# uclasystem/dorylus

Measured on AMD Instinct MI355X. Metric: full-graph GCN epoch: aggregated edges/sec (epoch time in ms_per_step), Reddit-scale synthetic, 2-layer 602-128-41, higher is better.
Workload: dtype f32

## Files before the change

dorylus_amd/_lib.py:

```python
import ctypes as C
import os

import numpy as np

_HERE = os.path.dirname(os.path.abspath(__file__))
LIB_PATH = os.environ.get("DORY_LIB_PATH") or os.path.join(_HERE, "libdorylus_hip.so")

SYMBOLS = [
    "dory_create", "dory_destroy", "dory_last_error", "dory_set_streams", "dory_sync",
    "dory_configure", "dory_graph_upload", "dory_preallocate", "dory_tensor_info",
    "dory_tensor_upload", "dory_tensor_download", "dory_tensor_fill_uniform", "dory_labels_upload",
    "dory_weight_set", "dory_weight_get", "dory_weight_grad_get", "dory_weight_grad_set", "dory_weights_init_xavier",
    "dory_aggregate", "dory_apply_vertex", "dory_apply_edge", "dory_predict_gat", "dory_train_stat", "dory_train_stat_global",
    "dory_halo_plan", "dory_comm_unique_id", "dory_comm_init", "dory_halo_exchange", "dory_halo_pack",
    "dory_halo_unpack", "dory_halo_pack_tensor", "dory_halo_unpack_tensor", "dory_adam_config", "dory_weight_update", "dory_timing_enable",
    "dory_timing_get", "dory_timing_reset", "dory_set_option", "dory_get_option", "dory_ctx_describe",
    "dory_epoch_graph_begin", "dory_epoch_graph_end", "dory_epoch_graph_launch", "dory_epoch_graph_drop",
    "dory_gatmh_heads", "dory_transform_first_active", "dory_transform_first_layer",
    "dory_comm_set_host_transport", "dory_comm_init_local", "dory_debug_occupy_cus",
]

ALLTOALLV_FN = C.CFUNCTYPE(C.c_int, C.c_void_p, C.POINTER(C.c_float), C.POINTER(C.c_uint64), C.POINTER(C.c_uint64),
                           C.POINTER(C.c_float), C.POINTER(C.c_uint64), C.POINTER(C.c_uint64), C.c_uint32)
ALLREDUCE_FN = C.CFUNCTYPE(C.c_int, C.c_void_p, C.POINTER(C.c_float), C.c_uint64)
# ... 56 lines not shown
        "dory_get_option": [vp, cp, C.POINTER(C.c_int64)],
        "dory_transform_first_active": [vp],
        "dory_transform_first_layer": [vp, u32],
        "dory_epoch_graph_begin": [vp], "dory_epoch_graph_end": [vp], "dory_epoch_graph_launch": [vp, u32],
        "dory_epoch_graph_drop": [vp],
        "dory_ctx_describe": [vp, C.POINTER(i32), C.POINTER(u32), C.POINTER(u32), C.POINTER(u32), C.POINTER(u32)],
        "dory_gatmh_heads": [vp, vp],
        "dory_comm_set_host_transport": [vp, ALLTOALLV_FN, ALLREDUCE_FN, vp],
        "dory_comm_init_local": [vp, C.c_uint32],
        "dory_partition_build": [vp, vp, u64, vp, u32, u32, u32, i32, C.POINTER(vp)],
        "dory_partition_build_from_files": [cp, u32, u32, i32, C.POINTER(vp)],
        "dory_partition_load": [cp, C.POINTER(vp)],
        "dory_partition_save": [vp, cp],
        "dory_partition_free": [vp],
        "dory_partition_get": [vp, vp],
        "dory_partition_upload": [vp, vp, vp],
        "dory_partition_recv_plan": [vp, vp, i32, vp, vp],
        "dory_partition_wire_order": [vp, vp, i32, vp, vp],
        "dory_read_layer_config": [cp, vp, u32, C.POINTER(u32)],
        "dory_read_features": [cp, vp, u32, u32, cp, vp, vp],
        "dory_read_labels": [cp, vp, u32, vp],
        "dory_engine_create": [vp, C.POINTER(vp)],
        "dory_engine_destroy": [vp],
        "dory_engine_run": [vp, u32, vp],
        "dory_engine_nn_compute": [vp, vp],
        "dory_engine_inc_layer": [vp, vp, vp],
        "dory_chunk_inc_layer": [i32, u32, vp, vp],
        "dory_engine_trace_epoch": [i32, u32, C.c_char_p, C.c_size_t],
        "dory_engine_is_last_layer": [vp, vp],
        "dory_engine_report": [vp, cp, C.c_size_t],
        "dory_sweep_deal": [u32, u32, u32, vp, vp, vp],
        "dory_sweep_deal_weighted": [u32, vp, u32, u32, u32, vp, vp, vp],
        "dory_sweep_geometry": [u32, u32, i32, i32, i32, u32, u32, u32, i32, vp],
    }
    for name, args in sig.items():
        if name in ("dory_partition_wire_order", "dory_sweep_geometry") and not hasattr(lib, name):
            continue
        fn = getattr(lib, name)
        fn.argtypes = args
        fn.restype = i32
    lib.dory_last_error.argtypes = [vp]
    lib.dory_last_error.restype = cp
    lib.dory_host_last_error.argtypes = []
    lib.dory_host_last_error.restype = cp
    lib.dory_formats_last_error.argtypes = []
    lib.dory_formats_last_error.restype = cp
    return lib


def _ptr(a):
    return a.ctypes.data_as(C.c_void_p) if a is not None else None


class Context:

    def __init__(self, device=0, lib=None):
        self.lib = lib or load()
        h = C.c_void_p()
        rc = self.lib.dory_create(device, C.byref(h))
        if rc != 0:
            raise DoryError(f"dory_create failed ({rc}): {self.lib.dory_last_error(None).decode()}")
        self.h = h
        self._keep = []

    def _ck(self, rc):
        if rc != 0:
            raise DoryError(f"dorylus_hip error {rc}: {self.lib.dory_last_error(self.h).decode()}")

    def close(self):
# ... 247 lines not shown
```

dorylus_amd/csrc/abi_context.hip:

```cpp
#include "abi_internal.hpp"

namespace dory {

static std::string g_create_err;

int fail(dory_ctx *c, int code, const char *fmt, ...) {
    char buf[512];
    va_list ap;
    va_start(ap, fmt);
    vsnprintf(buf, sizeof(buf), fmt, ap);
    va_end(ap);
    if (c) c->err = buf; else g_create_err = buf;
    return code;
}

void drain_timing(dory_ctx *c) {
    const dory_ctx::Pending *halo = nullptr;
    for (auto &p : c->pending) {
        (void)hipEventSynchronize(p.b);
        float ms = 0.f;
        if (hipEventElapsedTime(&ms, p.a, p.b) == hipSuccess) {
            c->times[p.fam].total_ms += ms;
            c->times[p.fam].launches += 1;
        }
// ... 156 lines not shown
int dory_create(int device, dory_ctx **out) {
    if (!out) return DORY_ERR_ARG;
    int n = 0;
    if (hipGetDeviceCount(&n) != hipSuccess || n == 0)
        return fail(nullptr, DORY_ERR_NODEVICE, "no HIP device visible (this library has no CPU fallback)");
    if (device < 0 || device >= n) return fail(nullptr, DORY_ERR_ARG, "device %d out of range (%d)", device, n);
    hipDeviceProp_t prop;
    if (hipGetDeviceProperties(&prop, device) != hipSuccess)
        return fail(nullptr, DORY_ERR_HIP, "hipGetDeviceProperties failed");
    if (!strstr(prop.gcnArchName, "gfx950"))
        return fail(nullptr, DORY_ERR_NODEVICE, "device %d is %s; kernels are built for gfx950 only", device,
                    prop.gcnArchName);
    dory_ctx *c = new dory_ctx();
    c->device = device;
    if (hipSetDevice(device) != hipSuccess || hipStreamCreateWithFlags(&c->compute, hipStreamNonBlocking) != hipSuccess ||
        hipStreamCreateWithFlags(&c->comm, hipStreamNonBlocking) != hipSuccess ||
        hipEventCreateWithFlags(&c->ev_a, hipEventDisableTiming) != hipSuccess ||
        hipEventCreateWithFlags(&c->ev_b, hipEventDisableTiming) != hipSuccess ||
        hipMalloc((void **)&c->d_stat, 2 * sizeof(float)) != hipSuccess ||
        hipMalloc((void **)&c->sweep_stat, SWEEP_STAT_WORDS * sizeof(uint32_t)) != hipSuccess ||
        hipMalloc((void **)&c->d_stat3, 256) != hipSuccess) {
        delete c;
        return fail(nullptr, DORY_ERR_HIP, "stream/event creation failed");
    }
    (void)hipMemset(c->d_stat, 0, 2 * sizeof(float));
    (void)hipMemset(c->sweep_stat, 0, SWEEP_STAT_WORDS * sizeof(uint32_t));
    c->own_compute = c->own_comm = true;
    c->opt["spmm_variant"] = 2;
    c->opt["spmm_sweep_flags"] = 0;
    c->opt["spmm_sweep_rows"] = 0;
    c->opt["spmm_sweep_pair"] = -1;
    c->opt["spmm_sweep_loader"] = 1;
    c->opt["spmm_sweep_loader_relief"] = 3;
    c->opt["spmm_sweep_reserve_cus"] = 4;
    c->opt["spmm_sweep_layout"] = 3;
    c->opt["spmm_sweep_window_kb"] = 0;
    c->cus_per_xcd = (uint32_t)std::max(1, prop.multiProcessorCount / 8);
    {
        const uint32_t PG = 2048;
        uint32_t *dx = nullptr;
        std::vector<uint32_t> hx(PG, 0xFFu);
        if (hipMalloc((void **)&dx, PG * sizeof(uint32_t)) == hipSuccess) {
            bool ran = launch_xcd_probe(dx, PG, c->compute) == hipSuccess && hipStreamSynchronize(c->compute) == hipSuccess &&
                       hipMemcpy(hx.data(), dx, PG * sizeof(uint32_t), hipMemcpyDeviceToHost) == hipSuccess;
            (void)hipFree(dx);
            uint32_t seen = 0, match = 0;
            for (uint32_t i = 0; i < PG; ++i) { if (hx[i] < 16) seen |= 1u << hx[i]; match += hx[i] == hx[i & 7u]; }
            uint32_t firsts = 0;
            for (uint32_t r = 0; r < 8; ++r) if (hx[r] < 16) firsts |= 1u << hx[r];
            c->xcd_count = (uint32_t)__builtin_popcount(seen);
            c->xcd_mapping_ok = ran && match == PG && c->xcd_count == 8 && __builtin_popcount(firsts) == 8;
        } else {
            c->xcd_mapping_ok = false;
        }
    }
    c->opt["spmm_xcd_assume_mismatch"] = 0;
    c->opt["spmm_slab"] = 0;
    c->opt["spmm_order"] = 1;
    c->opt["spmm_blk_group"] = 32;
    c->opt["spmm_blk_force_split"] = 0;
    c->opt["halo_overlap"] = 1;
    c->opt["gat_lazy_edge_tensors"] = 1;
    c->opt["gat_reuse_nsum"] = 1;
    c->opt["spmm_edge_split"] = 1;
    c->opt["spmm_sweep_cus"] = 0;
    c->opt["local_timeout_ms"] = 30000;
// ... 789 lines not shown
```

dorylus_amd/csrc/abi_stages.hip:

```cpp
#include "abi_internal.hpp"

namespace dory {
static BlockedAdj &gatmh_blocked_for(Adjacency &A, uint32_t ld) { return ld < 128 && A.blk16.built ? A.blk16 : A.blk; }

int ensure_blocked(dory_ctx *c, Adjacency &A, int group, bool narrow_set) {
    DerivedAdj &B = narrow_set ? A.blk16 : A.blk;
    const uint32_t want_nb = (uint32_t)c->opt["spmm_blk_nb"];
    const bool rebuild = B.built && want_nb && B.nb != (want_nb + 7) / 8 * 8;
    if (c->capturing && (!B.built || rebuild) && !A.blk.na)
        return fail(c, DORY_ERR_ARG, "epoch graph: blocked adjacency would have to be (re)built while recording");
    if (rebuild) {
        HIPCK(c, hipStreamSynchronize(c->compute));
        free_blocked(&B);
        B.built = false;
    }
    if (!B.built) {
        const uint32_t NG = c->N + A.ghosts;
        const uint64_t window = 0;
        const uint32_t nb = plan_blocks(NG, want_nb, (uint32_t)group * 16u, window);
        const bool tiny = !want_nb && (uint64_t)NG * group * 16u <= ((uint64_t)4 << 20) &&
                          !(c->gnn == DORY_GATMH && c->numNodes > 1);
        if (tiny || nb > 256 || (uint64_t)nb * (c->N + 1) * 8ull > ((uint64_t)8 << 30)) {
            if (!narrow_set) A.blk.na = true;
            return DORY_OK;
// ... 5 lines not shown
    return DORY_OK;
}

int ensure_sweep(dory_ctx *c, Adjacency &A, int group) {
    DerivedAdj &S = A.swp;
    const uint32_t want_nb = (uint32_t)c->opt["spmm_blk_nb"];
    if (S.built && S.want_nb != want_nb && !c->capturing) {
        HIPCK(c, hipStreamSynchronize(c->compute));
        free_blocked(&S);
        S.built = false;
    }
    if (S.built || S.na) return DORY_OK;
    if (c->capturing) return fail(c, DORY_ERR_ARG, "epoch graph: the sweep layout would have to be built while recording");
    const uint32_t NG = c->N + A.ghosts;
    int R;
    if (c->gnn == DORY_GATMH) {
        const uint32_t G_ = std::min<uint32_t>(32u, c->cus_per_xcd);
        const int forced = (int)c->opt["gatmh_sweep_rows"];
        R = (!forced && c->N >= 8u * G_ * 32u * 4u) ? 4 : sweep_pick_r(c->N, 32, G_, forced, 4);
    } else {
        R = sweep_pick_r(c->N, 32, std::min<uint32_t>(32u, c->cus_per_xcd), (int)c->opt["spmm_sweep_rows"]);
    }
    const bool out_edges = &A == &c->adj[ADJ_OUT];
    const uint64_t gat_kb = (c->gnn == DORY_GATMH && out_edges && c->opt["gatmh_src_window_kb"]) ? (uint64_t)c->opt["gatmh_src_window_kb"] : 4608u;
    const uint64_t window_kb = c->opt["spmm_sweep_window_kb"] ? (uint64_t)c->opt["spmm_sweep_window_kb"]
                                                              : (c->gnn == DORY_GATMH && R >= 4 ? gat_kb : (R <= 4 ? 3584u : 2432u));
    const uint64_t window = window_kb << 10;
    const uint64_t nb_est = ((uint64_t)NG * group * 16u + window - 1) / window + 1;
    const bool tiny = !want_nb && (uint64_t)NG * group * 16u <= ((uint64_t)4 << 20);
    if (tiny || c->N < 8 || (want_nb ? want_nb : nb_est) > 512 || (want_nb ? want_nb : nb_est) * (uint64_t)(c->N + 1) * 8ull > ((uint64_t)8 << 30)) {
        S.na = true;
        return DORY_OK;
    }
    HIPCK(c, build_blocked_sweep(A.ptr, A.idx, A.val, c->N, NG, A.nnz, want_nb, (uint32_t)group * 16u, window, R, &S, c->compute,
                                 (uint32_t)c->opt["spmm_sweep_layout"], std::min<uint32_t>(32u, c->cus_per_xcd),
                                 group == 32 && c->opt["spmm_sweep_loader"] ? (uint32_t)c->opt["spmm_sweep_loader_relief"] : 0u));
    S.want_nb = want_nb;
    S.built = true;
    return DORY_OK;
}

int blk_group_for(dory_ctx *c, uint32_t ld) {
    int group = (int)c->opt["spmm_blk_group"];
    if (group != 8 && group != 16 && group != 32) group = 32;
    if (ld < 128 && group == 32) group = 16;
    return group;
}

static int bf16_reserve(dory_ctx *c, uint64_t rows, uint32_t ld, const char *option) {
    const size_t need = (size_t)rows * ld * sizeof(uint16_t);
    if (need <= c->bf16_rows_bytes) return DORY_OK;
    if (c->capturing) return fail(c, DORY_ERR_ARG, "epoch graph: the bf16 rows of %s would have to grow while recording", option);
    if (c->bf16_rows) {
        HIPCK(c, hipStreamSynchronize(c->compute));
        (void)hipFree(c->bf16_rows);
        c->bf16_rows = nullptr;
        c->bf16_rows_bytes = 0;
        epoch_graph_drop_locked(c);
    }
    HIPCK(c, hipMalloc((void **)&c->bf16_rows, need));
    c->bf16_rows_bytes = need;
    return DORY_OK;
}
static int bf16_convert(dory_ctx *c, const Tensor &t, uint64_t first_row) {
    if (!t.rows) return DORY_OK;
    Timed tc(c, "bf16_convert", c->compute);
    HIPCK(c, launch_bf16_rows(t.d, c->bf16_rows + first_row * t.ld, t.rows * t.ld, c->compute));
    return DORY_OK;
}
// ... 775 lines not shown
```

dorylus_amd/csrc/ctx.hpp:

```cpp
#pragma once
#include <hip/hip_runtime.h>

#include <atomic>
#include <cstdint>
#include <map>
#include <memory>
#include <mutex>
#include <string>
#include <vector>

#include "../../include/dorylus_hip.h"
#include "sweep_geometry.hpp"

namespace dory {

struct Tensor {
    uint64_t rows = 0;
    uint32_t cols = 0;
    uint32_t ld = 0;
    float *d = nullptr;
    bool owned = true;
    size_t bytes() const { return (size_t)rows * ld * sizeof(float); }
};

// ... 210 lines not shown
    uint32_t N;
    uint32_t F;
    uint32_t ld;
    const uint64_t *ptr;
    const uint32_t *idx;
    const float *val;
    const float *self_scale;
    int self_mode;
    const float *xl;
    const float *xg;
    float *out;
    int accumulate;
    uint32_t row_clamp;
    uint32_t rows;
    const uint32_t *order;
    const uint64_t *ptr_end;
};
hipError_t launch_spmm(const SpmmArgs &a, int slab, hipStream_t s, bool bf16 = false);

void plan_long_rows(const uint64_t *ptr, uint32_t N, LongRowsHost *out);
hipError_t launch_spmm_long_rows(const SpmmArgs &a, const LongRowsDev &L, float *partial , hipStream_t s, bool bf16 = false);

hipError_t build_blocked(const uint64_t *ptr, const uint32_t *idx, const float *val, uint32_t N, uint32_t NG,
                         uint64_t nnz, uint32_t want_nb , uint32_t row_bytes, BlockedAdj *out,
                         hipStream_t s, uint64_t window_bytes = 0 );
uint32_t plan_blocks(uint32_t NG, uint32_t want_nb, uint32_t row_bytes, uint64_t window_bytes = 0);
hipError_t launch_spmm_blocked_part(const SpmmArgs &a, const BlockedAdj &B, float *partial, int group, bool unit,
                                    uint32_t b_lo, uint32_t b_hi, hipStream_t s);
hipError_t launch_spmm_blocked_long_segments(const SpmmArgs &a, const BlockedAdj &B, float *partial, bool unit,
                                             float *chunk_partial , hipStream_t s);
hipError_t launch_spmm_blocked_reduce(const SpmmArgs &a, const BlockedAdj &B, const float *partial,
                                      const float *row_scale, hipStream_t s);
void free_blocked(BlockedAdj *B);
hipError_t build_blocked_sweep(const uint64_t *ptr, const uint32_t *idx, const float *val, uint32_t N, uint32_t NG,
                               uint64_t nnz, uint32_t want_nb, uint32_t row_bytes, uint64_t window_bytes, int R,
                               BlockedAdj *out, hipStream_t s, uint32_t layout = 3 ,
                               uint32_t sweep_tiles = 32 ,
                               uint32_t loader_relief = 0 );
bool sweep_deal_plan(uint32_t nl, uint32_t R, uint32_t sweep_tiles, std::vector<uint32_t> *cap, uint32_t *npos, uint32_t loader_relief = 0);
bool sweep_deal_positions(uint32_t nl, uint32_t R, const std::vector<uint32_t> &cap, uint32_t *pos, uint32_t loader_lo = 0);
bool sweep_deal_balanced(uint32_t nl, uint32_t R, const std::vector<uint32_t> &cap, const uint64_t *w, uint32_t *pos);
int sweep_pick_r(uint32_t N, int group, uint32_t G, int force_r = 0 , int max_r = 10);
int sweep_rows(uint32_t rows_per_group, uint32_t npos, int group, uint32_t G, int force_r );
bool sweep_wide_rows_ok(int R);
SweepGeometry sweep_geometry(uint32_t npos, uint32_t ld, int group, int R, bool wide, uint32_t G);
size_t sweep_counter_bytes(const SweepGeometry &g, uint32_t nblocks);
size_t sweep_counter_bound(uint32_t npos, uint32_t ld, int group, int R, bool wide, uint32_t G, uint32_t nblocks);
bool sweep_supported(const SpmmArgs &a, const BlockedAdj &B, int group);
struct SweepCtl {
    int pair = -1;
    bool loader = true;
    uint32_t *stat = nullptr;
};
constexpr int SWEEP_STAT_WORDS = 8;
struct SweepPart {
    uint32_t cus;
    uint32_t b_lo, b_hi;
    bool accumulate;
    uint32_t reserve;
    int R;
    uint32_t *done;
    SweepCtl ctl;
    uint32_t flags;
    hipStream_t s;
    bool bf16;
    bool wide;
};
inline bool sweep_wide_applies(uint32_t ld, int group, int R16) { return ld >= 128 && (group == 16 || group == 32) && sweep_wide_rows_ok(R16); }
hipError_t launch_spmm_sweep(SpmmArgs a, const BlockedAdj &B, int group, const float *row_scale, float *split_partial, const SweepPart &p);
hipError_t launch_spmm_sweep_combine(const SpmmArgs &a, const BlockedAdj &B, const float *row_scale, const float *split_partial,
                                     hipStream_t s, bool bf16 = false);
hipError_t launch_bf16_rows(const float *x, uint16_t *y, uint64_t n, hipStream_t s);
hipError_t launch_occupy_cus(uint32_t workgroups, uint64_t usec, hipStream_t s);
hipError_t launch_xcd_probe(uint32_t *xcc , uint32_t grid, hipStream_t s);
// ... 159 lines not shown
```

dorylus_amd/csrc/spmm.hip:

```cpp
#include <algorithm>
#include <cmath>
#include <vector>

#include "sweep_core.hpp"

namespace dory {

template <int GROUP, int CHUNKS, bool BF16>
__device__ __forceinline__ void spmm_rows_body(SpmmArgs a) {
    typedef RowChunk<BF16> RC;
    constexpr int RPW = 64 / GROUP;
    constexpr int RPB = 4 * RPW;
    const int lane = threadIdx.x & 63;
    const int wave = threadIdx.x >> 6;
    const int li = lane % GROUP;
    const int gi = lane / GROUP;
    const uint32_t rid = blockIdx.x * RPB + wave * RPW + gi;
    const bool row_ok = rid < (a.rows ? a.rows : a.N);
    uint32_t v = row_ok ? (a.order ? a.order[rid] : rid) : 0;
    if constexpr (GROUP == 64)
        v = (uint32_t)__builtin_amdgcn_readfirstlane((int)v);

    const uint32_t nchunk = a.ld >> 2;
    const uint32_t c0 = blockIdx.y * (GROUP * CHUNKS) + li;
    bool act[CHUNKS];
    uint32_t col[CHUNKS];
    float4 acc[CHUNKS];
#pragma unroll
    for (int k = 0; k < CHUNKS; ++k) {
        act[k] = row_ok && (c0 + GROUP * k) < nchunk;
        col[k] = act[k] ? c0 + GROUP * k : 0;
        acc[k] = make_float4(0.f, 0.f, 0.f, 0.f);
    }
    if (a.accumulate == 2) {
// ... 342 lines not shown
        }
        if (a.self_mode != 0) {
            const float sc = a.self_mode == 1 ? a.self_scale[v] : 1.f;
            acc = fma4(sc, row_chunk(xl4[(size_t)v * nchunk + col]), acc);
        }
        if (a.accumulate) {
            const float4 p = out4[col];
            acc.x += p.x; acc.y += p.y; acc.z += p.z; acc.w += p.w;
        }
        out4[col] = acc;
    }
}
__global__ __launch_bounds__(320) void spmm_sweep_combine_kernel(SpmmArgs a, BlockedAdj B, const float *row_scale,
                                                                 const float *split_partial, uint32_t tpr) {
    spmm_sweep_combine_body<false>(a, B, row_scale, split_partial, tpr);
}
__global__ __launch_bounds__(320) void spmm_sweep_combine_bf16_kernel(SpmmArgs a, BlockedAdj B, const float *row_scale,
                                                                      const float *split_partial, uint32_t tpr) {
    spmm_sweep_combine_body<true>(a, B, row_scale, split_partial, tpr);
}

hipError_t launch_spmm_sweep_combine(const SpmmArgs &a, const BlockedAdj &B, const float *row_scale, const float *split_partial,
                                     hipStream_t s, bool bf16) {
    if (!B.nsplit || a.ld == 0) return hipSuccess;
    const uint32_t nchunk = a.ld >> 2;
    const uint32_t tpr = std::min<uint32_t>(256u, (nchunk + 31u) & ~31u);
    const uint32_t rpb = std::max<uint32_t>(1u, 320u / tpr);
    hipLaunchKernelGGL(bf16 ? spmm_sweep_combine_bf16_kernel : spmm_sweep_combine_kernel, dim3((B.nsplit + rpb - 1) / rpb),
                       dim3(tpr * rpb), 0, s, a, B, row_scale, split_partial, tpr);
    return hipGetLastError();
}

constexpr uint32_t SWEEP_SPLIT = 2;

hipError_t build_blocked_sweep(const uint64_t *ptr, const uint32_t *idx, const float *val, uint32_t N, uint32_t NG,
                               uint64_t nnz, uint32_t want_nb, uint32_t row_bytes, uint64_t window_bytes, int R,
                               BlockedAdj *out, hipStream_t s, uint32_t layout, uint32_t sweep_tiles, uint32_t loader_relief) {
    BlockedAdj B{};
    if (N == 0 || NG == 0) { *out = B; return hipSuccess; }
    hipError_t e;
#define BCK(x) if ((e = (x)) != hipSuccess) return e
    std::vector<uint64_t> hptr((size_t)N + 1);
    BCK(hipMemcpyAsync(hptr.data(), ptr, ((size_t)N + 1) * sizeof(uint64_t), hipMemcpyDeviceToHost, s));
    BCK(hipStreamSynchronize(s));
    const uint64_t split_deg = std::max<uint64_t>(64, (uint64_t)SWEEP_SPLIT * (nnz / N + 1));
    struct Item { uint32_t row, k, K; uint64_t w; };
    std::vector<Item> items;
    items.reserve(N);
    std::vector<uint32_t> split_rows;
    uint32_t nslots = 0;
    for (uint32_t v = 0; v < N; ++v) {
        const uint64_t deg = hptr[v + 1] - hptr[v];
        if (deg > split_deg) {
            const uint64_t K64 = (deg + split_deg - 1) / split_deg;
            if (K64 > 0x7FFFFFFFull || (uint64_t)nslots + K64 > 0x7FFFFFFFull) return hipErrorInvalidValue;
            const uint32_t K = (uint32_t)K64;
            split_rows.insert(split_rows.end(), {v, nslots, K});
            for (uint32_t k = 0; k < K; ++k) items.push_back({v, k, K, (deg + K - 1) / K});
            nslots += K;
        } else {
            items.push_back({v, 0, 1, deg});
        }
    }
    if (layout & 2u) std::stable_sort(items.begin(), items.end(), [](const Item &x, const Item &y) { return x.w > y.w; });
    const uint64_t ni64 = items.size();
    if (ni64 + 16 > 0xFFFFFFF0ull) return hipErrorInvalidValue;
    const uint32_t nl = (uint32_t)ni64;
    uint32_t npos = std::max<uint32_t>((nl + R - 1) / (uint32_t)R * (uint32_t)R, 8);
    std::vector<uint32_t> ipos(nl);
    if (layout & 2u) {
// ... 53 lines not shown
    B.SB = (std::max(N, G) + std::max(nbL, std::max<uint32_t>(nbG, 1)) - 1) / std::max(nbL, std::max<uint32_t>(nbG, 1));
    B.npos = npos;
    B.nb_local = nbL;
    B.nghost = G;
    B.rows_per_group = (uint32_t)R;
    B.row_bytes = row_bytes;
    uint32_t *cnt = nullptr;
    uint16_t *d_sblk = nullptr;
    uint64_t *dtotal = nullptr;
    BCK(hipMalloc((void **)&B.perm, (size_t)npos * sizeof(uint32_t)));
    BCK(hipMemcpyAsync(B.perm, perm.data(), (size_t)npos * sizeof(uint32_t), hipMemcpyHostToDevice, s));
    BCK(hipMalloc((void **)&d_sblk, (size_t)NG * sizeof(uint16_t)));
    BCK(hipMemcpyAsync(d_sblk, sblk.data(), (size_t)NG * sizeof(uint16_t), hipMemcpyHostToDevice, s));
    uint2 *d_slice = nullptr;
    if (nslots) {
        BCK(hipMalloc((void **)&B.otgt, (size_t)npos * sizeof(uint32_t)));
        BCK(hipMemcpyAsync(B.otgt, otgt.data(), (size_t)npos * sizeof(uint32_t), hipMemcpyHostToDevice, s));
        BCK(hipMalloc((void **)&d_slice, (size_t)npos * sizeof(uint2)));
        BCK(hipMemcpyAsync(d_slice, slice.data(), (size_t)npos * sizeof(uint2), hipMemcpyHostToDevice, s));
        BCK(hipMalloc((void **)&B.split_rows, split_rows.size() * sizeof(uint32_t)));
        BCK(hipMemcpyAsync(B.split_rows, split_rows.data(), split_rows.size() * sizeof(uint32_t), hipMemcpyHostToDevice, s));
        B.nsplit = (uint32_t)(split_rows.size() / 3);
        B.nslots = nslots;
    }
    BCK(hipMalloc((void **)&cnt, (size_t)nb * npos * sizeof(uint32_t)));
    BCK(hipMemsetAsync(cnt, 0, (size_t)nb * npos * sizeof(uint32_t), s));
    BCK(hipMalloc((void **)&B.boff, (size_t)nb * (npos + 1) * sizeof(uint32_t)));
    BCK(hipMalloc((void **)&B.bbase, (size_t)(nb + 1) * sizeof(uint64_t)));
    BCK(hipMalloc((void **)&B.bent, (nnz + 130) * sizeof(uint2)));
    BCK(hipMemsetAsync(B.bent + nnz, 0, 130 * sizeof(uint2), s));
    BCK(hipMalloc((void **)&dtotal, nb * sizeof(uint64_t)));
    hipLaunchKernelGGL(blk_count_kernel, dim3((npos + 255) / 256), dim3(256), 0, s, npos, ptr, idx, B.SB, cnt, B.perm, d_sblk,
                       (const uint2 *)d_slice);
    hipLaunchKernelGGL(blk_scan_kernel, dim3(nb), dim3(1024), 0, s, npos, cnt, B.boff, dtotal);
    std::vector<uint64_t> tot(nb), base(nb + 1, 0);
    BCK(hipMemcpyAsync(tot.data(), dtotal, nb * sizeof(uint64_t), hipMemcpyDeviceToHost, s));
    BCK(hipStreamSynchronize(s));
    for (uint32_t b = 0; b < nb; ++b) base[b + 1] = base[b] + tot[b];
    if (base[nb] != nnz) return hipErrorUnknown;
    BCK(hipMemcpyAsync(B.bbase, base.data(), (nb + 1) * sizeof(uint64_t), hipMemcpyHostToDevice, s));
    hipLaunchKernelGGL(blk_fill_kernel, dim3((npos + 255) / 256), dim3(256), 0, s, npos, nb, ptr, idx, val, B.SB, B.bbase,
                       B.boff, cnt, (uint32_t *)nullptr, (float *)nullptr, B.perm, d_sblk, (const uint2 *)d_slice, B.bent);
    BCK(hipGetLastError());
    BCK(hipStreamSynchronize(s));
    (void)hipFree(cnt);
    (void)hipFree(dtotal);
    (void)hipFree(d_sblk);
    if (d_slice) (void)hipFree(d_slice);
#undef BCK
    *out = B;
    return hipSuccess;
}

bool sweep_supported(const SpmmArgs &a, const BlockedAdj &B, int group) {
    const uint64_t row_b = (uint64_t)a.ld * 4u;
    const bool addr_ok = (uint64_t)a.N * row_b < (1ull << 32) && (uint64_t)B.nghost * row_b < (1ull << 32) &&
                         (uint64_t)a.N + B.nghost < (1u << 24) && row_b < (1u << 24);
    return (group == 16 || group == 32) && !(a.ld & 3) && B.nb > 0 && B.nchunks == 0 && a.N >= 8 && B.npos >= 8 && addr_ok;
}

hipError_t sweep_plan(const SpmmArgs &a, const BlockedAdj &B, int group, const SweepPart &p, float *split_partial, SweepPlan *pl) {
    if (!sweep_supported(a, B, group) || p.b_hi > B.nb || p.cus == 0 || p.cus > 32 || !p.ctl.stat) return hipErrorInvalidValue;
    if (p.b_lo < B.nb_local && p.b_hi > B.nb_local) return hipErrorInvalidValue;
    if (p.b_lo >= B.nb_local && !a.xg) return hipErrorInvalidValue;
    const uint32_t G = p.cus > 12 ? p.cus - std::min<uint32_t>(p.reserve, 8u) : p.cus;
    const SweepGeometry g = sweep_geometry(B.npos, a.ld, group, p.R, p.wide, G);
    const uint32_t flags = p.flags | (p.accumulate ? 2u : 0u) | (p.reserve ? 32u : 0u);
    *pl = SweepPlan{SweepArgs{g.rpx, g.tiles_x, G, g.nsweeps, p.b_lo, p.b_hi, p.done, flags, split_partial, p.ctl.stat}, dim3(g.grid_x), g.slabs};
    return hipMemsetAsync(p.done, 0, sweep_counter_bytes(g, p.b_hi - p.b_lo), p.s);
}

template <class F>
static bool k1s_narrow_form(int group, int R, F f) {
    if (group == 32) return sweep_pick<2, 4, 6, 8, 10>(R, [&](auto RR) { return f(std::integral_constant<int, 32>{}, RR); });
    return group == 16 && sweep_pick<2, 3, 4, 5, 6, 8>(R, [&](auto RR) { return f(std::integral_constant<int, 16>{}, RR); });
}

hipError_t launch_spmm_sweep(SpmmArgs a, const BlockedAdj &B, int group, const float *row_scale, float *split_partial, const SweepPart &p) {
    if (a.N == 0 || a.ld == 0 || p.b_lo >= p.b_hi) return hipSuccess;
    if (p.bf16 && row_scale) return hipErrorInvalidValue;
    if (p.wide && (!p.bf16 || (a.ld & 7) || !sweep_wide_applies(a.ld, group, p.R))) return hipErrorInvalidValue;
    if (B.nslots && !split_partial) return hipErrorInvalidValue;
    if (p.accumulate) { a.self_mode = 0; a.accumulate = 1; }
    SweepPlan pl;
    const hipError_t e = sweep_plan(a, B, group, p, split_partial, &pl);
    if (e != hipSuccess) return e;
    const dim3 bl(SWEEP_NT);
    const bool unit = row_scale != nullptr;
    const bool pair = (p.R & 1) ? false : (p.ctl.pair < 0 ? pl.slabs >= 3 : p.ctl.pair != 0);
    const bool found = p.wide ? sweep_pick<2, 3, 4, 5>(p.R, [&](auto R) {
        return sweep_pick<0, 1>(p.ctl.loader, [&](auto L) {
            hipLaunchKernelGGL((spmm_sweep_bf16x8_kernel<R(), L() != 0>), pl.grid, bl, 0, p.s, a, B, pl.w);
            return true;
        });
    }) : k1s_narrow_form(group, p.R, [&](auto G, auto R) {
        return sweep_pick<0, 1>(p.ctl.loader, [&](auto L) {
            return sweep_pick<0, 1>(pair, [&](auto P) {
                hipLaunchKernelGGL((p.bf16 ? spmm_sweep_bf16_kernel<G(), R(), false, P() != 0, L() != 0>
                                    : unit ? spmm_sweep_kernel<G(), R(), true, P() != 0, L() != 0>
                                           : spmm_sweep_kernel<G(), R(), false, P() != 0, L() != 0>), pl.grid, bl, 0, p.s, a, B, row_scale, pl.w);
                return true;
            });
        });
    });
    return found ? hipGetLastError() : hipErrorInvalidValue;
}

__global__ __launch_bounds__(1024) void occupy_cus_kernel(uint64_t ticks, uint32_t *sink) {
    extern __shared__ uint32_t occupy_lds[];
    asm volatile("v_mov_b32 v127, 0" ::: "v127");
    const uint64_t t0 = wall_clock64();
    while (wall_clock64() - t0 < ticks) __builtin_amdgcn_s_sleep(64);
    if (ticks == ~0ull) { occupy_lds[threadIdx.x] = 1; sink[0] = occupy_lds[0]; }
}
hipError_t launch_occupy_cus(uint32_t workgroups, uint64_t usec, hipStream_t s) {
    if (!workgroups) return hipSuccess;
    hipError_t e = hipFuncSetAttribute(reinterpret_cast<const void *>(occupy_cus_kernel), hipFuncAttributeMaxDynamicSharedMemorySize, 96 << 10);
    if (e != hipSuccess) return e;
    hipLaunchKernelGGL(occupy_cus_kernel, dim3(workgroups), dim3(1024), 96 << 10, s, usec * 100ull, (uint32_t *)nullptr);
    return hipGetLastError();
}

// ... 11 lines not shown
```

dorylus_amd/host/sweep_deal.cpp:

```cpp
#include <algorithm>
#include <cstdint>
#include <vector>

#include "../../include/dorylus_host.h"

namespace dory {

bool sweep_deal_plan(uint32_t nl, uint32_t R, uint32_t sweep_tiles, std::vector<uint32_t> *cap, uint32_t *npos,
                     uint32_t loader_relief) {
    if (R == 0) return false;
    loader_relief = std::min(loader_relief, R / 2);
    const uint32_t tiles = std::max<uint32_t>(1, sweep_tiles);
    const uint32_t GS = tiles * 32u;
    const uint32_t n_x = (nl + 7) / 8;
    auto relief_of = [&](uint32_t rows) { return (uint32_t)(((uint64_t)loader_relief * rows + R / 2) / R); };
    auto capacity = [&](uint32_t need) -> uint64_t {
        const uint32_t S = (need + R - 1) / R, last = need - (S - 1) * R;
        const uint64_t full = (uint64_t)GS * R - (uint64_t)2 * tiles * relief_of(R);
        const uint64_t tail = (uint64_t)GS * last - (uint64_t)2 * tiles * std::min(relief_of(last), last);
        return (uint64_t)(S - 1) * full + tail;
    };
    uint32_t need = std::max<uint32_t>(1, (n_x + GS - 1) / GS);
    const uint32_t S_plain = (need + R - 1) / R;
    for (;; --loader_relief) {
        need = std::max<uint32_t>(1, (n_x + GS - 1) / GS);
        while (capacity(need) < n_x) ++need;
        if ((need + R - 1) / R == S_plain || loader_relief == 0) break;
    }
    const uint32_t S = (need + R - 1) / R;
    if ((uint64_t)8 * S * GS * R > 0xFFFFFFF0ull) return false;
    const uint32_t T = 8u * S * GS;
    const uint32_t last = need - (S - 1) * R;
    cap->assign(T, R);
    for (uint32_t x = 0; x < 8; ++x)
// ... 37 lines not shown
    }
    return i == nl;
}

bool sweep_deal_balanced(uint32_t nl, uint32_t R, const std::vector<uint32_t> &cap, const uint64_t *w, uint32_t *pos) {
    const uint32_t T = (uint32_t)cap.size();
    struct Node { uint64_t load; uint32_t cap, g; };
    auto worse = [](const Node &a, const Node &b) {
        const unsigned __int128 l = (unsigned __int128)a.load * b.cap, r = (unsigned __int128)b.load * a.cap;
        return l != r ? l > r : a.g > b.g;
    };
    std::vector<Node> heap;
    heap.reserve(T);
    for (uint32_t g = 0; g < T; ++g)
        if (cap[g]) heap.push_back({0, cap[g], g});
    std::make_heap(heap.begin(), heap.end(), worse);
    std::vector<uint32_t> used(T, 0);
    for (uint32_t i = 0; i < nl; ++i) {
        if (heap.empty()) return false;
        std::pop_heap(heap.begin(), heap.end(), worse);
        Node n = heap.back();
        heap.pop_back();
        if (used[n.g] >= R) return false;
        pos[i] = n.g * R + used[n.g]++;
        n.load += w[i];
        if (used[n.g] < cap[n.g]) {
            heap.push_back(n);
            std::push_heap(heap.begin(), heap.end(), worse);
        }
    }
    return heap.empty();
}

}

extern "C" int dory_sweep_deal(uint32_t items, uint32_t rows_per_group, uint32_t sweep_tiles, uint32_t *positions_out,
                               uint32_t *group_rows_out, uint32_t *item_position) {
    std::vector<uint32_t> cap;
    uint32_t npos = 0;
    if (!dory::sweep_deal_plan(items, rows_per_group, sweep_tiles, &cap, &npos, 0)) return 1;
    if (positions_out) *positions_out = npos;
    if (group_rows_out) std::copy(cap.begin(), cap.end(), group_rows_out);
    if (item_position && !dory::sweep_deal_positions(items, rows_per_group, cap, item_position, 0)) return 2;
    return 0;
}

extern "C" int dory_sweep_deal_weighted(uint32_t items, const uint64_t *weights, uint32_t rows_per_group, uint32_t sweep_tiles,
                                        uint32_t loader_relief, uint32_t *positions_out, uint32_t *group_rows_out,
                                        uint32_t *item_position) {
    if (!weights) return 1;
    std::vector<uint32_t> cap;
    uint32_t npos = 0;
    if (!dory::sweep_deal_plan(items, rows_per_group, sweep_tiles, &cap, &npos, loader_relief)) return 1;
    if (positions_out) *positions_out = npos;
    if (group_rows_out) std::copy(cap.begin(), cap.end(), group_rows_out);
    if (item_position && !dory::sweep_deal_balanced(items, rows_per_group, cap, weights, item_position)) return 2;
    return 0;
}
```

include/dorylus_host.h:

```cpp
#ifndef DORYLUS_HOST_H
#define DORYLUS_HOST_H

#include <stddef.h>
#include <stdint.h>

#include "dorylus_hip.h"

#ifdef __cplusplus
extern "C" {
#endif

typedef struct dory_partition dory_partition;

int dory_partition_build(const uint32_t *src, const uint32_t *dst, uint64_t num_records,
                         const int32_t *parts, uint32_t global_vtx_cnt, uint32_t node_id,
                         uint32_t num_nodes, int undirected, dory_partition **out);
int dory_partition_build_from_files(const char *dataset_dir, uint32_t node_id, uint32_t num_nodes,
                                    int undirected, dory_partition **out);
int dory_partition_load(const char *graph_bin_path, dory_partition **out);
int dory_partition_save(const dory_partition *p, const char *graph_bin_path);
int dory_partition_free(dory_partition *p);
const char *dory_host_last_error(void);

struct dory_partition_view {
// ... 21 lines not shown

int dory_partition_wire_order(const dory_partition *p, const int32_t *parts, int dir, uint32_t *order, uint32_t *idxs);

int dory_partition_upload(dory_ctx *ctx, const dory_partition *p, const int32_t *parts);

int dory_read_layer_config(const char *path, uint32_t *dims, uint32_t max_dims, uint32_t *count);
int dory_read_features(const char *path, const dory_partition *p, uint32_t expect_dim, uint32_t node_id,
                       const char *cache_dir, float *local, float *ghost);
int dory_read_labels(const char *path, const dory_partition *p, uint32_t expect_kinds, uint32_t *labels);
const char *dory_formats_last_error(void);

typedef struct dory_engine dory_engine;
int dory_engine_create(dory_ctx *ctx, dory_engine **out);
int dory_engine_destroy(dory_engine *e);
int dory_engine_run(dory_engine *e, uint32_t epochs, double *epoch_ms);
struct dory_chunk {
    uint32_t localId, globalId, lowBound, upBound, layer;
    int32_t dir;
    uint32_t epoch;
    uint8_t vertex;
};
int dory_engine_nn_compute(dory_engine *e, struct dory_chunk *chunk);
int dory_engine_inc_layer(dory_engine *e, const struct dory_chunk *in, struct dory_chunk *out);
int dory_engine_is_last_layer(dory_engine *e, const struct dory_chunk *c);
int dory_chunk_inc_layer(int gnn_type, uint32_t num_layers, const struct dory_chunk *in, struct dory_chunk *out);
int dory_engine_trace_epoch(int gnn_type, uint32_t num_layers, char *buf, size_t buflen);
int dory_engine_report(dory_engine *e, char *buf, size_t buflen);

int dory_sweep_deal(uint32_t items, uint32_t rows_per_group, uint32_t sweep_tiles, uint32_t *positions_out,
                    uint32_t *group_rows_out, uint32_t *item_position);
int dory_sweep_deal_weighted(uint32_t items, const uint64_t *weights, uint32_t rows_per_group, uint32_t sweep_tiles,
                             uint32_t loader_relief, uint32_t *positions_out, uint32_t *group_rows_out,
                             uint32_t *item_position);
int dory_sweep_geometry(uint32_t positions, uint32_t ld, int group, int rows, int wide, uint32_t cus, uint32_t nblocks,
                        uint32_t layout_rows, int rows_option, uint64_t *out);

#ifdef __cplusplus
}
#endif
#endif
```

Before: 18.91 billion.

## Rearrange sweep SpMM row positions within waves to balance lockstep block costs

Adds a host-side local search that permutes row positions within each wave of the blocked sweep SpMM layout. Rows that execute in lockstep, singly or in pairs, then get similar per-block nonzero counts, which cuts the padding and idle lanes caused by uneven rows. The search is weighted by how many layers use paired or plain sweep launches. It runs once at adjacency build time, adding a device-to-host copy of the counts, multithreaded CPU work, and a recount. It is enabled by default for plain fp32 GCN.

```diff
diff --git a/dorylus_amd/_lib.py b/dorylus_amd/_lib.py
--- a/dorylus_amd/_lib.py
+++ b/dorylus_amd/_lib.py
@@ -112,9 +112,10 @@
         "dory_sweep_deal": [u32, u32, u32, vp, vp, vp],
         "dory_sweep_deal_weighted": [u32, vp, u32, u32, u32, vp, vp, vp],
         "dory_sweep_geometry": [u32, u32, i32, i32, i32, u32, u32, u32, i32, vp],
+        "dory_sweep_arrange": [u32, u32, u32, vp, vp, u32, u32, u32, u32, u32, vp, vp],
     }
     for name, args in sig.items():
-        if name in ("dory_partition_wire_order", "dory_sweep_geometry") and not hasattr(lib, name):
+        if name in ("dory_partition_wire_order", "dory_sweep_geometry", "dory_sweep_arrange") and not hasattr(lib, name):
             continue
         fn = getattr(lib, name)
         fn.argtypes = args
diff --git a/dorylus_amd/csrc/abi_context.hip b/dorylus_amd/csrc/abi_context.hip
--- a/dorylus_amd/csrc/abi_context.hip
+++ b/dorylus_amd/csrc/abi_context.hip
@@ -212,6 +212,7 @@
     c->opt["spmm_sweep_pair"] = -1;
     c->opt["spmm_sweep_loader"] = 1;
     c->opt["spmm_sweep_loader_relief"] = 3;
+    c->opt["spmm_sweep_arrange"] = -1;
     c->opt["spmm_sweep_reserve_cus"] = 4;
     c->opt["spmm_sweep_layout"] = 3;
     c->opt["spmm_sweep_window_kb"] = 0;
diff --git a/dorylus_amd/csrc/abi_stages.hip b/dorylus_amd/csrc/abi_stages.hip
--- a/dorylus_amd/csrc/abi_stages.hip
+++ b/dorylus_amd/csrc/abi_stages.hip
@@ -61,9 +61,28 @@
         S.na = true;
         return DORY_OK;
     }
+    const int64_t arr_opt = c->opt["spmm_sweep_arrange"];
+    SweepArrange arr{0, 0, arr_opt == 2};
+    const bool plain_fp32 = c->gnn != DORY_GATMH && !c->opt["gcn_bf16_gather"] && !c->opt["gcn_bf16_wide"];
+    if (arr_opt > 0 || (arr_opt < 0 && plain_fp32)) {
+        const int64_t pair_opt = c->opt["spmm_sweep_pair"];
+        auto launch = [&](uint32_t cols) {
+            const uint32_t ld = pad_ld(cols);
+            if (blk_group_for(c, ld) != 32) return;
+            const uint32_t slabs = ((ld >> 2) + 31u) / 32u;
+            (sweep_rows_in_pairs(R, slabs, pair_opt) ? arr.w_pair : arr.w_plain) += slabs;
+        };
+        for (uint32_t l = 0; l < c->L; ++l) {
+            if (c->gnn != DORY_GCN) launch(c->dims[l + 1]);
+            else if (tf_layer(c, l)) launch(c->dims[l + 1]);
+            else if (!out_edges || l >= 1) launch(c->dims[l]);
+        }
+        if (!arr.w_pair && !arr.w_plain) arr.w_plain = 1;
+    }
     HIPCK(c, build_blocked_sweep(A.ptr, A.idx, A.val, c->N, NG, A.nnz, want_nb, (uint32_t)group * 16u, window, R, &S, c->compute,
                                  (uint32_t)c->opt["spmm_sweep_layout"], std::min<uint32_t>(32u, c->cus_per_xcd),
-                                 group == 32 && c->opt["spmm_sweep_loader"] ? (uint32_t)c->opt["spmm_sweep_loader_relief"] : 0u));
+                                 group == 32 && c->opt["spmm_sweep_loader"] ? (uint32_t)c->opt["spmm_sweep_loader_relief"] : 0u,
+                                 (arr.w_pair || arr.w_plain) ? &arr : nullptr));
     S.want_nb = want_nb;
     S.built = true;
     return DORY_OK;
diff --git a/dorylus_amd/csrc/ctx.hpp b/dorylus_amd/csrc/ctx.hpp
--- a/dorylus_amd/csrc/ctx.hpp
+++ b/dorylus_amd/csrc/ctx.hpp
@@ -266,14 +266,24 @@
 hipError_t launch_spmm_blocked_reduce(const SpmmArgs &a, const BlockedAdj &B, const float *partial,
                                       const float *row_scale, hipStream_t s);
 void free_blocked(BlockedAdj *B);
+inline bool sweep_rows_in_pairs(int R, uint32_t slabs, int64_t pair_opt) {
+    return (R & 1) ? false : (pair_opt < 0 ? slabs >= 3 : pair_opt != 0);
+}
+struct SweepArrange {
+    uint32_t w_pair, w_plain;
+    bool report;
+};
 hipError_t build_blocked_sweep(const uint64_t *ptr, const uint32_t *idx, const float *val, uint32_t N, uint32_t NG,
                                uint64_t nnz, uint32_t want_nb, uint32_t row_bytes, uint64_t window_bytes, int R,
                                BlockedAdj *out, hipStream_t s, uint32_t layout = 3 ,
                                uint32_t sweep_tiles = 32 ,
-                               uint32_t loader_relief = 0 );
+                               uint32_t loader_relief = 0 ,
+                               const SweepArrange *arrange = nullptr );
 bool sweep_deal_plan(uint32_t nl, uint32_t R, uint32_t sweep_tiles, std::vector<uint32_t> *cap, uint32_t *npos, uint32_t loader_relief = 0);
 bool sweep_deal_positions(uint32_t nl, uint32_t R, const std::vector<uint32_t> &cap, uint32_t *pos, uint32_t loader_lo = 0);
 bool sweep_deal_balanced(uint32_t nl, uint32_t R, const std::vector<uint32_t> &cap, const uint64_t *w, uint32_t *pos);
+bool sweep_arrange(uint32_t nb, uint32_t npos, uint32_t R, const uint32_t *counts, const uint8_t *occupied, uint32_t U, uint32_t w_pair,
+                   uint32_t w_plain, bool exact_tail, uint32_t threads, uint32_t *from, uint64_t *cost);
 int sweep_pick_r(uint32_t N, int group, uint32_t G, int force_r = 0 , int max_r = 10);
 int sweep_rows(uint32_t rows_per_group, uint32_t npos, int group, uint32_t G, int force_r );
 bool sweep_wide_rows_ok(int R);
diff --git a/dorylus_amd/csrc/spmm.hip b/dorylus_amd/csrc/spmm.hip
--- a/dorylus_amd/csrc/spmm.hip
+++ b/dorylus_amd/csrc/spmm.hip
@@ -1,5 +1,9 @@
 #include <algorithm>
+#include <chrono>
 #include <cmath>
+#include <cstdio>
+#include <cstdlib>
+#include <thread>
 #include <vector>
 
 #include "sweep_core.hpp"
@@ -408,10 +412,12 @@
 }
 
 constexpr uint32_t SWEEP_SPLIT = 2;
+constexpr uint64_t SWEEP_ARRANGE_MAX_BYTES = (uint64_t)256 << 20;
 
 hipError_t build_blocked_sweep(const uint64_t *ptr, const uint32_t *idx, const float *val, uint32_t N, uint32_t NG,
                                uint64_t nnz, uint32_t want_nb, uint32_t row_bytes, uint64_t window_bytes, int R,
-                               BlockedAdj *out, hipStream_t s, uint32_t layout, uint32_t sweep_tiles, uint32_t loader_relief) {
+                               BlockedAdj *out, hipStream_t s, uint32_t layout, uint32_t sweep_tiles, uint32_t loader_relief,
+                               const SweepArrange *arrange) {
     BlockedAdj B{};
     if (N == 0 || NG == 0) { *out = B; return hipSuccess; }
     hipError_t e;
@@ -531,6 +537,47 @@
     BCK(hipMalloc((void **)&dtotal, nb * sizeof(uint64_t)));
     hipLaunchKernelGGL(blk_count_kernel, dim3((npos + 255) / 256), dim3(256), 0, s, npos, ptr, idx, B.SB, cnt, B.perm, d_sblk,
                        (const uint2 *)d_slice);
+    if (arrange && (layout & 2u) && (arrange->w_pair || arrange->w_plain) && R > 2 &&
+        (uint64_t)nb * npos * sizeof(uint32_t) <= SWEEP_ARRANGE_MAX_BYTES) {
+        const auto t0 = std::chrono::steady_clock::now();
+        std::vector<uint32_t> hcnt((size_t)nb * npos), from(npos);
+        BCK(hipMemcpyAsync(hcnt.data(), cnt, (size_t)nb * npos * sizeof(uint32_t), hipMemcpyDeviceToHost, s));
+        BCK(hipStreamSynchronize(s));
+        std::vector<uint8_t> occ(npos);
+        for (uint32_t p = 0; p < npos; ++p) occ[p] = perm[p] != 0xFFFFFFFFu;
+        uint32_t threads = std::max(1u, std::min(16u, std::thread::hardware_concurrency()));
+        if (const char *ev = getenv("DORY_BUILD_THREADS")) threads = (uint32_t)std::max(1, std::min(16, atoi(ev)));
+        uint64_t cost[6] = {0, 0, 0, 0, 0, 0};
+        if (!sweep_arrange(nb, npos, (uint32_t)R, hcnt.data(), occ.data(), K1S_BATCH, arrange->w_pair, arrange->w_plain, false,
+                           threads, from.data(), cost)) cost[5] = 0;
+        if (cost[5]) {
+            const std::vector<uint32_t> perm0 = perm, otgt0 = otgt;
+            const std::vector<uint2> slice0 = slice;
+            for (uint32_t p = 0; p < npos; ++p) {
+                perm[p] = perm0[from[p]];
+                if (nslots) { otgt[p] = otgt0[from[p]]; slice[p] = slice0[from[p]]; }
+            }
+            BCK(hipMemcpyAsync(B.perm, perm.data(), (size_t)npos * sizeof(uint32_t), hipMemcpyHostToDevice, s));
+            if (nslots) {
+                BCK(hipMemcpyAsync(B.otgt, otgt.data(), (size_t)npos * sizeof(uint32_t), hipMemcpyHostToDevice, s));
+                BCK(hipMemcpyAsync(d_slice, slice.data(), (size_t)npos * sizeof(uint2), hipMemcpyHostToDevice, s));
+            }
+            BCK(hipMemsetAsync(cnt, 0, (size_t)nb * npos * sizeof(uint32_t), s));
+            hipLaunchKernelGGL(blk_count_kernel, dim3((npos + 255) / 256), dim3(256), 0, s, npos, ptr, idx, B.SB, cnt, B.perm, d_sblk,
+                               (const uint2 *)d_slice);
+            BCK(hipStreamSynchronize(s));
+        }
+        if (arrange->report) {
+            const double ms = std::chrono::duration<double, std::milli>(std::chrono::steady_clock::now() - t0).count();
+            const double ideal = std::max<double>(1.0, (double)cost[4] / 2.0);
+            fprintf(stderr, "sweep_arrange: %u blocks x %u positions, R %d, batch %d, weights pairs %u plain %u: pairs %llu -> %llu "
+                            "(x ideal %.4f -> %.4f), plain %llu -> %llu (x ideal %.4f -> %.4f); %llu entries, %llu waves changed, "
+                            "%.1f ms on %u threads\n",
+                    nb, npos, R, (int)K1S_BATCH, arrange->w_pair, arrange->w_plain, (unsigned long long)cost[0], (unsigned long long)cost[1],
+                    cost[0] / ideal, cost[1] / ideal, (unsigned long long)cost[2], (unsigned long long)cost[3], cost[2] / ideal,
+                    cost[3] / ideal, (unsigned long long)cost[4], (unsigned long long)cost[5], ms, threads);
+        }
+    }
     hipLaunchKernelGGL(blk_scan_kernel, dim3(nb), dim3(1024), 0, s, npos, cnt, B.boff, dtotal);
     std::vector<uint64_t> tot(nb), base(nb + 1, 0);
     BCK(hipMemcpyAsync(tot.data(), dtotal, nb * sizeof(uint64_t), hipMemcpyDeviceToHost, s));
@@ -586,7 +633,7 @@
     if (e != hipSuccess) return e;
     const dim3 bl(SWEEP_NT);
     const bool unit = row_scale != nullptr;
-    const bool pair = (p.R & 1) ? false : (p.ctl.pair < 0 ? pl.slabs >= 3 : p.ctl.pair != 0);
+    const bool pair = sweep_rows_in_pairs(p.R, pl.slabs, p.ctl.pair);
     const bool found = p.wide ? sweep_pick<2, 3, 4, 5>(p.R, [&](auto R) {
         return sweep_pick<0, 1>(p.ctl.loader, [&](auto L) {
             hipLaunchKernelGGL((spmm_sweep_bf16x8_kernel<R(), L() != 0>), pl.grid, bl, 0, p.s, a, B, pl.w);
diff --git a/dorylus_amd/host/sweep_deal.cpp b/dorylus_amd/host/sweep_deal.cpp
--- a/dorylus_amd/host/sweep_deal.cpp
+++ b/dorylus_amd/host/sweep_deal.cpp
@@ -1,5 +1,6 @@
 #include <algorithm>
 #include <cstdint>
+#include <thread>
 #include <vector>
 
 #include "../../include/dorylus_host.h"
@@ -103,6 +104,125 @@
     return heap.empty();
 }
 
+constexpr uint32_t ARRANGE_ROUNDS = 12;
+
+namespace {
+struct ArrangeModel { uint32_t U; bool exact; };
+inline uint32_t lockstep_cost(uint32_t a, uint32_t b, const ArrangeModel &m) {
+    const uint32_t fa = a / m.U, fb = b / m.U, ra = a % m.U, rb = b % m.U;
+    const uint32_t tail = m.exact ? std::max(ra, rb) : ((ra | rb) ? m.U - 1 : 0u);
+    return m.U * std::max(fa, fb) + tail;
+}
+struct WaveCost {
+    const uint32_t *c;
+    const uint32_t *row;
+    uint32_t R, nb;
+    ArrangeModel m;
+    const uint32_t *at(uint32_t h, uint32_t s) const { return c + (size_t)row[h * R + s] * nb; }
+    uint64_t plain(uint32_t s) const {
+        const uint32_t *a = at(0, s), *b = at(1, s);
+        uint64_t t = 0;
+        for (uint32_t k = 0; k < nb; ++k) t += lockstep_cost(a[k], b[k], m);
+        return t;
+    }
+    uint64_t pair(uint32_t rr) const {
+        const uint32_t *a0 = at(0, 2 * rr), *a1 = at(0, 2 * rr + 1), *b0 = at(1, 2 * rr), *b1 = at(1, 2 * rr + 1);
+        uint64_t t = 0;
+        for (uint32_t k = 0; k < nb; ++k) t += lockstep_cost(a0[k] + a1[k], b0[k] + b1[k], m);
+        return t;
+    }
+};
+}
+
+bool sweep_arrange(uint32_t nb, uint32_t npos, uint32_t R, const uint32_t *counts, const uint8_t *occupied, uint32_t U,
+                   uint32_t w_pair, uint32_t w_plain, bool exact_tail, uint32_t threads, uint32_t *from, uint64_t *cost) {
+    if (R == 0 || U == 0 || npos % R || !from || (nb && npos && (!counts || !occupied))) return false;
+    for (uint32_t p = 0; p < npos; ++p) from[p] = p;
+    const uint32_t W = 2 * R, nwaves = npos / W;
+    const bool pairs = !(R & 1u);
+    if (!pairs) w_pair = 0;
+    const bool arrange = R > 2 && (w_pair || w_plain);
+    threads = std::max<uint32_t>(1, std::min<uint32_t>(threads, 16));
+    threads = std::min<uint32_t>(threads, std::max<uint32_t>(1, nwaves));
+    std::vector<uint64_t> acc((size_t)threads * 6, 0);
+    auto work = [&](uint32_t t) {
+        std::vector<uint32_t> c((size_t)W * nb), row(W), occ;
+        std::vector<uint64_t> pc(R), qc(R / 2 + 1);
+        uint64_t *out = &acc[(size_t)t * 6];
+        const uint32_t w_lo = (uint32_t)((uint64_t)nwaves * t / threads), w_hi = (uint32_t)((uint64_t)nwaves * (t + 1) / threads);
+        for (uint32_t w = w_lo; w < w_hi; ++w) {
+            const uint32_t p0 = w * W;
+            for (uint32_t b = 0; b < nb; ++b)
+                for (uint32_t i = 0; i < W; ++i) {
+                    const uint32_t v = counts[(size_t)b * npos + p0 + i];
+                    c[(size_t)i * nb + b] = v;
+                    out[4] += v;
+                }
+            occ.clear();
+            uint32_t in_half[2] = {0, 0};
+            for (uint32_t i = 0; i < W; ++i) {
+                row[i] = i;
+                if (occupied[p0 + i]) { occ.push_back(i); ++in_half[i / R]; }
+            }
+            WaveCost wc{c.data(), row.data(), R, nb, ArrangeModel{U, exact_tail}};
+            uint64_t plain = 0, pair = 0;
+            for (uint32_t s = 0; s < R; ++s) plain += pc[s] = wc.plain(s);
+            if (pairs) for (uint32_t rr = 0; rr < R / 2; ++rr) pair += qc[rr] = wc.pair(rr);
+            out[0] += pair; out[2] += plain;
+            bool changed = false;
+            if (arrange && in_half[0] && in_half[1]) {
+                for (uint32_t round = 0; round < ARRANGE_ROUNDS; ++round) {
+                    bool kept = false;
+                    for (size_t x = 0; x + 1 < occ.size(); ++x)
+                        for (size_t y = x + 1; y < occ.size(); ++y) {
+                            const uint32_t i = occ[x], j = occ[y], si = i % R, sj = j % R;
+                            if (si == sj) continue;
+                            std::swap(row[i], row[j]);
+                            const uint64_t pi = w_plain ? wc.plain(si) : 0, pj = w_plain ? wc.plain(sj) : 0;
+                            const bool two = si / 2 != sj / 2;
+                            const uint64_t qi = w_pair ? wc.pair(si / 2) : 0, qj = (w_pair && two) ? wc.pair(sj / 2) : 0;
+                            const uint64_t before = (uint64_t)w_plain * (pc[si] + pc[sj]) + (uint64_t)w_pair * (qc[si / 2] + (two ? qc[sj / 2] : 0));
+                            const uint64_t after = (uint64_t)w_plain * (pi + pj) + (uint64_t)w_pair * (qi + qj);
+                            if (after < before) {
+                                if (w_plain) { pc[si] = pi; pc[sj] = pj; }
+                                if (w_pair) { qc[si / 2] = qi; if (two) qc[sj / 2] = qj; }
+                                kept = changed = true;
+                            } else {
+                                std::swap(row[i], row[j]);
+                            }
+                        }
+                    if (!kept) break;
+                }
+            }
+            plain = pair = 0;
+            for (uint32_t s = 0; s < R; ++s) plain += wc.plain(s);
+            if (pairs) for (uint32_t rr = 0; rr < R / 2; ++rr) pair += wc.pair(rr);
+            out[1] += pair; out[3] += plain; out[5] += changed;
+            for (uint32_t i = 0; i < W; ++i) from[p0 + i] = p0 + row[i];
+        }
+    };
+    if (threads == 1) {
+        work(0);
+    } else {
+        std::vector<std::thread> pool;
+        for (uint32_t t = 0; t < threads; ++t) pool.emplace_back(work, t);
+        for (auto &th : pool) th.join();
+    }
+    if (cost)
+        for (uint32_t k = 0; k < 6; ++k) {
+            cost[k] = 0;
+            for (uint32_t t = 0; t < threads; ++t) cost[k] += acc[(size_t)t * 6 + k];
+        }
+    return true;
+}
+
+}
+
+extern "C" int dory_sweep_arrange(uint32_t blocks, uint32_t positions, uint32_t rows_per_group, const uint32_t *counts,
+                                  const uint8_t *occupied, uint32_t batch, uint32_t weight_pair, uint32_t weight_plain,
+                                  uint32_t exact_tail, uint32_t threads, uint32_t *from_position, uint64_t *cost) {
+    return dory::sweep_arrange(blocks, positions, rows_per_group, counts, occupied, batch, weight_pair, weight_plain,
+                               exact_tail != 0, threads, from_position, cost) ? 0 : 1;
 }
 
 extern "C" int dory_sweep_deal(uint32_t items, uint32_t rows_per_group, uint32_t sweep_tiles, uint32_t *positions_out,
diff --git a/include/dorylus_host.h b/include/dorylus_host.h
--- a/include/dorylus_host.h
+++ b/include/dorylus_host.h
@@ -77,6 +77,9 @@
 int dory_sweep_deal_weighted(uint32_t items, const uint64_t *weights, uint32_t rows_per_group, uint32_t sweep_tiles,
                              uint32_t loader_relief, uint32_t *positions_out, uint32_t *group_rows_out,
                              uint32_t *item_position);
+int dory_sweep_arrange(uint32_t blocks, uint32_t positions, uint32_t rows_per_group, const uint32_t *counts,
+                       const uint8_t *occupied, uint32_t batch, uint32_t weight_pair, uint32_t weight_plain,
+                       uint32_t exact_tail, uint32_t threads, uint32_t *from_position, uint64_t *cost);
 int dory_sweep_geometry(uint32_t positions, uint32_t ld, int group, int rows, int wide, uint32_t cus, uint32_t nblocks,
                         uint32_t layout_rows, int rows_option, uint64_t *out);
 
```

Result: no change. 19.09 billion, median of 6 (+0.9%).
